# toverainc/willow-inference-server

Measured on AMD Instinct MI355X. Metric: realtime_multiple (audio_ms / infer_ms), Whisper large-v2 beam=5, 3.84 s clip, higher is better.
Workload: dtype f16; 1 GPU; whisper-large beam=5 clip=3sec (3840 ms) batch=1/GPU, PCM resident in HBM -> ids on host; parallelism=1 independent replicas (utterance sharding, no data-path collective)

## Files before the change

### include/wis_hip.h

```cpp
#ifndef WIS_HIP_H
#define WIS_HIP_H

#include <stddef.h>
#include <stdint.h>

#ifdef __cplusplus
extern "C" {
#endif

#define WIS_ABI_VERSION 1

#define WIS_OK             0
#define WIS_E_ARG         -1
#define WIS_E_FORMAT      -2
#define WIS_E_NOMEM       -3
#define WIS_E_CHECKSUM    -4
#define WIS_E_HIP         -5
#define WIS_E_STATE       -6
#define WIS_E_UNSUPPORTED -7

#define WIS_SAMPLE_RATE 16000
#define WIS_N_FFT       400
#define WIS_HOP         160
#define WIS_N_MELS      80
// ... 118 lines not shown
int wis_debug_align_matrix(wis_model_t* m, const float* input, int input_kind, int B, const int32_t* start_seq, int P,
                           const int32_t* text, const int32_t* text_len, const int32_t* num_frames, int median_filter_width, float* out);
int wis_align_last_timing(wis_model_t* m, float* ms);
int wis_op_dtw(int device, const float* x, int N, int M, int32_t* text_idx, int32_t* time_idx, int32_t* len);
int wis_op_align_matrix(int device, const float* q, const void* kx_f16, int T_tokens, int n_heads_sel, int T, int frames, int width, float* out);
int wis_debug_tree_logits(wis_model_t* m, const float* input, int input_kind, const int32_t* prompt, int P, int beam,
                          const int32_t* tok, const int32_t* org, int n_steps, float* logits);

int wis_debug_search(wis_model_t* m, const float* logits, int n_steps, int B, const wis_gen_opts_t* opts,
                     int32_t* out_ids, int32_t* out_len, float* out_score, int32_t* out_finish_step, int32_t* out_parent);
int wis_debug_search_n(wis_model_t* m, const float* logits, int n_steps, int B, const wis_gen_opts_t* opts, const uint64_t* seeds, const uint32_t* noise,
                       int32_t* out_ids, int32_t* out_len, float* out_score, int32_t* out_finish_step, int32_t* out_parent);

int wis_debug_handoff(wis_model_t* m, int raise_flag, int* retries, int* spin_disabled);
int wis_debug_graph_count(wis_model_t* m, int* count);
int wis_debug_sa_long(wis_model_t* m, int form);

typedef struct {
  float logmel_ms, encoder_ms, crosskv_ms, prefill_ms, decode_ms, total_ms;
  int32_t decode_steps;
  int32_t decode_steps_needed;
} wis_timing_t;
int wis_last_timing(const wis_model_t* m, wis_timing_t* t);

int wis_debug_phase_cycles(wis_model_t* m, int B, int beam, int pos, uint64_t* out);

int wis_debug_timeline(wis_model_t* m, int B, int beam, int pos, int use_graph, uint64_t* out, int n_out);
int wis_debug_sampling_cycles(wis_model_t* m, uint64_t* out);

int wis_bench_weight_stream(wis_model_t* m, int M, int passes, float* total_ms, int* launches_per_pass,
// ... 105 lines not shown
```

### willow-inference-server_amd/csrc/generate.hip

```cpp
#include <math.h>
#include <stdlib.h>
#include <string.h>
#include <time.h>
#include <algorithm>
#include <chrono>
#include <cmath>
#include <vector>

#include "common.hpp"
#include "kernels.hpp"
#include "model.hpp"

using namespace wis;

namespace {

struct SampleCtx {
  wis_model* m; hipStream_t st;
  int B, P, beam;
  SampleCfg sc; const float* bias_all;
  bool ts; int ts_max_init;
  float rep_pen = 1.f; int rep_ngram = 0;
  bool rep() const { return rep_pen != 1.f || rep_ngram != 0; }
  SampleP sp;
// ... 106 lines not shown
      for (int r = 0; r < B * beam; ++r) { ht[r] = r; ht[MAX_ROWS + r] = r / beam * beam; }
      WIS_HIP_CHECK(hipMemcpyAsync(m->d_sa_tab, ht, sizeof(m->h_pin->sa_tab), hipMemcpyHostToDevice, g.st));
    }
  } else
  if (!g.drafting || g.beam_draft) {
    std::vector<int> tok(B * P), pos(B * P), slot(B * P), ls(B * P);
    for (int b = 0; b < B; ++b) for (int i = 0; i < P; ++i) { tok[b * P + i] = g.prompt[b * P + i]; pos[b * P + i] = i; slot[b * P + i] = b * beam; ls[b * P + i] = b * beam; }
    WIS_RET(upload_rows(m, tok, pos, slot, ls, false));
  }
  if (m->overrun_left) { WIS_HIP_CHECK(hipMemsetAsync(m->ca_epoch, 0, 4, g.st)); m->overrun_left = false; }
  __atomic_store_n(&m->h_prog[HP_REC], 0ull, __ATOMIC_RELAXED);
  m->h_prog[HP_DONE_STEP] = 0; m->h_prog[HP_DONE_STAMP] = 0; m->h_prog[HP_STAMP0] = 0;
  return WIS_OK;
}

static int front_half(const GenCtx& g) {
  wis_model* m = g.m; hipStream_t st = g.st; const int B = g.B;
  static const bool one_stream = getenv("WIS_ONE_STREAM") != nullptr;
  static const bool two_streams = getenv("WIS_TWO_STREAMS") != nullptr;
  const bool alone = g_active_calls[m->device & 63].load(std::memory_order_relaxed) <= 1;
  hipStream_t se = (one_stream || !(alone || two_streams)) ? st : m->st_enc;
  if (se != st) WIS_HIP_CHECK(hipStreamWaitEvent(se, m->ev_ckv, 0));
  WIS_HIP_CHECK(hipEventRecord(m->ev[0], se));
  WIS_RET(stage_input(m, g.input, g.o->input_kind, B, se));
  WIS_HIP_CHECK(hipEventRecord(m->ev[1], se));
  WIS_RET(run_encoder(m, B, se));
  WIS_HIP_CHECK(hipEventRecord(m->ev[2], se));
  if (se != st) { WIS_HIP_CHECK(hipEventRecord(m->ev_enc, se)); WIS_HIP_CHECK(hipStreamWaitEvent(st, m->ev_enc, 0)); }
  WIS_RET(run_cross_kv(m, B));
  WIS_HIP_CHECK(hipEventRecord(m->ev[3], st));
  WIS_HIP_CHECK(hipEventRecord(m->ev_ckv, st));
  return WIS_OK;
}

struct LogitRows { int b, j, off; };
enum { TAIL_TAPS = 1, TAIL_NO_CACHE = 2 };
static int sampling_tail(const SampleCtx& g, LogitRows rows, int flags) {
  wis_model* m = g.m; hipStream_t st = g.st; const wis_config_t& c = m->cfg;
  const int lr_b = rows.b, lr_j = rows.j, lr_off = rows.off;
  unsigned long long* prof = (WIS_TAPS && (flags & TAIL_TAPS)) ? m->d_prof + (size_t)c.n_dec_layers * 8 * 16 : nullptr;
  if (g.rep()) WIS_RET(launch_rep_rules(st, m->logits, m->bs, g.B, g.sc, g.rep_pen, g.rep_ngram, lr_b, lr_j, lr_off));
  if (g.ts) WIS_RET(launch_ts_rules(st, m->logits, g.bias_all, m->bias_begin, m->bs, g.B, g.sc, c.no_timestamps, g.ts_max_init, lr_b, lr_j, lr_off, m->ts_desc));
  if (g.sampling()) {
    WIS_RET(launch_logit_stats(st, m->logits, g.bias_all, m->bias_begin, m->bs.step_u, m->st_max, m->st_sum, m->st_val, m->st_idx, g.B, g.sc, lr_b, lr_j, lr_off, nullptr,
// ... 22 lines not shown
  explicit TicketScope(wis_model* mm) : m(mm), spin_call(mm->spin_now) { m->spin_now = false; }
  ~TicketScope() { m->spin_now = spin_call; }
};

static int reseed_tick(wis_model* m, int steps) {
  unsigned* tk = m->h_pin->reseed_tick;
  tk[0] = (unsigned)steps; tk[1] = m->gen; tk[2] = 0; tk[3] = 0;
  WIS_HIP_CHECK(hipMemcpyAsync(m->bs.tick, tk, 16, hipMemcpyHostToDevice, m->st));
  return WIS_OK;
}

static void pack_traj(int* hd, const int32_t* tok, const int32_t* org, int n, int k) {
  for (int s_ = 0; s_ < n; ++s_) for (int j = 0; j < k; ++j) { hd[(s_ * MAX_R + j) * 2] = tok[s_ * k + j]; hd[(s_ * MAX_R + j) * 2 + 1] = org[s_ * k + j]; }
}

static int seed_prefill(const GenCtx& g) {
  wis_model* m = g.m; const wis_config_t& c = m->cfg; const int B = g.B, P = g.P;
  WIS_RET(dec_forward(m, B * P, P, B, true, g.beam, 0));
  if (g.sot_row >= 0) WIS_RET(launch_no_speech(g.st, m->logits, m->n_vocab_pad, B, P, g.sot_row, c.n_vocab, c.no_speech, m->d_nsp));
  return sampling_tail(g, {P, 0, P - 1}, TAIL_TAPS);
}

static int seed_prefill_long(const GenCtx& g) {
  wis_model* m = g.m; hipStream_t st = g.st; const wis_config_t& c = m->cfg; PinnedScratch* hp = m->h_pin;
  const int B = g.B, P = g.P, beam = g.beam, Pl = g.Pl, Np = P - Pl, G = MAX_ROWS / 16;
  for (int ub0 = 0; ub0 < B; ub0 += G) {
    const int nb = std::min(G, B - ub0), M = nb * 16;
    for (int r = 0; r < M; ++r) hp->base[r] = hp->anc[r] = (ub0 + r / 16) * beam;
    WIS_HIP_CHECK(hipMemcpyAsync(m->d_anc, hp->anc, (size_t)M * 4, hipMemcpyHostToDevice, st));
    WIS_HIP_CHECK(hipMemcpyAsync(m->d_base, hp->base, (size_t)M * 4, hipMemcpyHostToDevice, st));
    for (int t0 = 0; t0 < Np; t0 += 16) {
      const int n = std::min(16, Np - t0);
      std::vector<int> tok(M), pos(M), slot(M), ls(M);
      for (int r = 0; r < M; ++r) {
        const int u = ub0 + r / 16, i = std::min(r % 16, n - 1);
// ... 174 lines not shown
  ~StepGraph() { g.m->sa_nb = 8; }

  int nb_for(int passes_done) const {
    static const bool sa_short = !(getenv("WIS_SA_NB") && atoi(getenv("WIS_SA_NB")) == 0);
    const int len = g.P + passes_done;
    return (!sa_short || g.long_p) ? 8 : (len <= 16 ? 2 : (len <= 32 ? 4 : 8));
  }
  int one_step() const {
    g.m->sa_plen = g.plen; g.m->sa_w0 = g.P;
    const int rc = dec_forward(g.m, g.B * g.beam, g.beam, g.B, true, g.beam, 1);
    g.m->sa_plen = nullptr;
    WIS_RET(rc);
    return sampling_tail(g, {g.beam, 1, 0}, TAIL_TAPS | (g.sampling() ? TAIL_NO_CACHE : 0));
  }
  int graph_for(int nb, hipGraphExec_t* out) const {
    wis_model* m = g.m; const SampleCfg& sc = g.sc;
    GraphKey key; memset(&key, 0, sizeof(key));
    key.B = g.B; key.beam = g.beam; key.P = (g.long_p && sa_long_kernel(m)) ? -1 : g.P ; key.max_new = g.max_new; key.fixed_new = sc.fixed_new; key.suppress_blank = sc.suppress_blank;
    key.suppress_default = g.o->suppress_default; key.early_exit = sc.allow_early_exit; key.lp = sc.length_penalty; key.patience = g.patience; key.spin = m->spin_now ? 1 : 0;
    key.sa_nb = nb;
    key.timestamps = g.ts ? 1 : 0; key.max_init = g.ts ? g.ts_max_init : 0;
    key.rep_pen = g.rep_pen == 1.f ? 0.f : g.rep_pen; key.rep_ngram = g.rep_ngram;
    key.samp_topk = g.sp.topk; key.samp_T = g.sampling() ? g.sp.T : 0.f; key.n_hyp = g.n_res > 1 ? g.n_res : 0;
    auto it = m->graphs.find(key);
    if (it != m->graphs.end()) { *out = it->second; return WIS_OK; }
    hipGraph_t graph = nullptr; hipGraphExec_t ge = nullptr;
    WIS_HIP_CHECK(hipStreamBeginCapture(g.st, hipStreamCaptureModeThreadLocal));
    int rc = one_step();
    hipError_t e = hipStreamEndCapture(g.st, &graph);
    if (rc) { if (graph) hipGraphDestroy(graph); return rc; }
    if (e != hipSuccess) { set_error("graph capture failed: %s", hipGetErrorString(e)); return WIS_E_HIP; }
    e = hipGraphInstantiate(&ge, graph, nullptr, nullptr, 0);
    hipGraphDestroy(graph);
    if (e != hipSuccess) { set_error("graph instantiate failed: %s", hipGetErrorString(e)); return WIS_E_HIP; }
    m->graphs[key] = ge;
    *out = ge;
    return WIS_OK;
  }
// ... 1 lines not shown
    wis_model* m = g.m;
    m->sa_nb = nb_for(passes_done);
    if (!m->use_graph) return one_step();
    hipGraphExec_t ge = nullptr;
    WIS_RET(graph_for(m->sa_nb, &ge));
    WIS_HIP_CHECK(hipGraphLaunch(ge, g.st));
    return WIS_OK;
  }
};

struct LoopResult {
  int steps;
  int needed = 0;
  bool gave_up = false;
  bool from_host = false;
  float decode_ms_dev = -1.f;
};
static void unpack_progress(const wis_model* m, int* st_, int* dn_, int* gu_) {
  const unsigned long long r = __atomic_load_n(&m->h_prog[HP_REC], __ATOMIC_ACQUIRE);
  if ((r >> 48) != (unsigned long long)m->gen) { *st_ = 0; *dn_ = 0; *gu_ = 0; return; }
  *st_ = (int)((r >> 32) & 0xFFFFu); *gu_ = (int)((r >> 16) & 0xFFFFu); *dn_ = (int)(r & 0xFFFFu);
}
static int check_terminated(const GenCtx& g, LoopResult* lr, int dn_, int gu_) {
  lr->gave_up = gu_ != 0;
  if (!lr->gave_up && dn_ < g.B) { set_error("decode did not terminate within %d steps (done %d of %d)", lr->steps, dn_, g.B); return WIS_E_STATE; }
  return WIS_OK;
}

static inline void cpu_relax() {
#if !defined(__HIP_DEVICE_COMPILE__) && defined(__x86_64__)
  __builtin_ia32_pause();
#endif
}

static int run_burst(const GenCtx& g, const StepGraph& sg, int limit, LoopResult* lr) {
  wis_model* m = g.m;
  for (; lr->steps < limit; ++lr->steps) WIS_RET(sg.launch_pass(lr->steps));
  WIS_HIP_CHECK(hipEventRecord(m->ev[5], g.st));
  WIS_HIP_CHECK(hipStreamSynchronize(g.st));
  int st_, dn_, gu_; unpack_progress(m, &st_, &dn_, &gu_);
  WIS_RET(check_terminated(g, lr, dn_, gu_));
  lr->needed = lr->steps;
  return WIS_OK;
}

static int run_paced(const GenCtx& g, const StepGraph& sg, int limit, int base_done, LoopResult* lr) {
  wis_model* m = g.m; const int B = g.B;
  int& steps = lr->steps;
  const auto t_dec0 = std::chrono::steady_clock::now();
  const int depth = g.o->queue_depth > 0 ? g.o->queue_depth : 2;
  auto t_last = std::chrono::steady_clock::now();
  int seen = -1, st_ = 0, dn_ = 0, gu_ = 0;
  static const bool trace = getenv("WIS_EOT_TRACE") != nullptr;
  struct Tr { int step; unsigned long long dev; double host_us; int launched; };
  std::vector<Tr> tr;
  const auto t_loop = std::chrono::steady_clock::now();
  for (unsigned spins = 0;; ++spins) {
// ... 19 lines not shown
    }
    cpu_relax();
  }
  if (trace) {
    unsigned long long prev_dev = 0;
    for (size_t i = 0; i < tr.size(); ++i) {
      if (tr[i].step < 0) { fprintf(stderr, "[eot-trace]   launch of step %d took the host %.1f us\n", -tr[i].step, tr[i].host_us); continue; }
      fprintf(stderr, "[eot-trace] step %d seen by the host at %.1f us (device clock +%.1f us since the previous record), %d steps enqueued\n", tr[i].step, tr[i].host_us,
              prev_dev ? (double)(tr[i].dev - prev_dev) * 0.01 : 0.0, tr[i].launched);
      prev_dev = tr[i].dev;
    }
    fprintf(stderr, "[eot-trace] done seen at %.1f us: %d of %d utterances, %d steps enqueued\n", std::chrono::duration<double, std::micro>(std::chrono::steady_clock::now() - t_loop).count(), dn_, B, steps);
  }
  WIS_RET(check_terminated(g, lr, dn_, gu_));
  if (!lr->gave_up) {
    lr->from_host = true;
    lr->needed = (int)m->h_prog[HP_DONE_STEP];
    const unsigned long long s0 = m->h_prog[HP_STAMP0], s1 = m->h_prog[HP_DONE_STAMP];
    lr->decode_ms_dev = s1 > s0 ? (float)((double)(s1 - s0) * 1e-5) : 0.f;
    if (g.drafting) lr->decode_ms_dev = std::chrono::duration<float, std::milli>(std::chrono::steady_clock::now() - t_dec0).count();
  }
  return WIS_OK;
}

static void results_from_verification(const GenCtx& g, const Seed& sd, int32_t* out_ids, int32_t* out_len, float* out_score) {
  float sfin = sd.spec_cum;
  if (g.sc.length_penalty != 0.f) sfin /= powf((float)sd.spec_len, g.sc.length_penalty);
  out_len[0] = sd.spec_len;
  for (int t = 0; t < g.max_new; ++t) out_ids[t] = t < sd.spec_len ? sd.spec_gen[t] : 0;
  if (out_score) out_score[0] = sfin;
}
// ... 39 lines not shown
  m->timing.decode_steps_needed = lr.needed;
}

static int generate_impl(wis_model_t* m, const float* input, int B, const int32_t* prompt, int P,
                 const wis_gen_opts_t* o, int32_t* out_ids, int32_t* out_len, float* out_score, bool* retry,
                 const int32_t* draft = nullptr, int n_draft = 0, int* accepted = nullptr, const int32_t* draft_org = nullptr,
                 const uint64_t* seeds = nullptr, bool single = true) {
  *retry = false;
  if (accepted) *accepted = 0;
  m->nsp_B = 0;
  WIS_HIP_CHECK(hipSetDevice(m->device));
  SpinClaim claim(m, B);
  GenCtx g;
  WIS_RET(make_gen_ctx(m, input, B, prompt, P, o, draft, n_draft, draft_org, seeds, single, &g));
  hipStream_t st = g.st;
  WIS_RET(stage_search(g));
  WIS_RET(front_half(g));

  Seed sd;
  if (g.long_p) WIS_RET(seed_prefill_long(g));
  else if (!g.drafting) WIS_RET(seed_prefill(g));
  else {
    TicketScope ticket(m);
    WIS_RET(g.beam_draft ? seed_beam_draft(g, &sd) : seed_greedy_draft(g, &sd));
    if (accepted) *accepted = sd.accepted;
  }
  WIS_HIP_CHECK(hipEventRecord(m->ev[4], st));
  if (sd.beam_fin) WIS_HIP_CHECK(hipEventRecord(m->ev[5], st));

  const StepGraph sg{g};
  LoopResult lr; lr.steps = sd.steps;
  const int known = (g.sc.fixed_new > 0) ? std::min(g.max_new, g.sc.fixed_new + 1) : 0;
  if (sd.spec_done || sd.beam_fin) lr.needed = sd.steps;
  else if (known) WIS_RET(run_burst(g, sg, known, &lr));
  else WIS_RET(run_paced(g, sg, g.max_new, g.drafting ? sd.steps : 0, &lr));
  if (lr.gave_up) {
    WIS_HIP_CHECK(hipMemsetAsync(m->ca_epoch, 0, 4, st));
    WIS_HIP_CHECK(hipStreamSynchronize(st));
    m->spin_off = true; *retry = true; ++m->handoff_retries;
    fprintf(stderr, "[wis_hip] device %d: decoder cross-attention granule hand-off timed out; this handle uses the ticket hand-off from now on, the call is repeated\n", m->device);
    return WIS_OK;
  }
  if (sd.spec_done) { results_from_verification(g, sd, out_ids, out_len, out_score); lr.from_host = true; lr.decode_ms_dev = 0.f; }
  else if (lr.from_host) WIS_RET(results_from_record(g, out_ids, out_len, out_score));
  else WIS_RET(results_from_device(m, B * g.n_res, g.max_new, out_ids, out_len, out_score));
  record_timing(g, lr);
  if (lr.steps > lr.needed) { claim.defer(st); m->overrun_left = true; }
  if (g.sot_row >= 0) m->nsp_B = B;
  return WIS_OK;
}

static int generate_with_retry(const char* who, wis_model_t* m, const float* input, int B, const int32_t* prompt, int P, const wis_gen_opts_t* o,
                               int32_t* out_ids, int32_t* out_len, float* out_score,
                               const int32_t* draft = nullptr, int n_draft = 0, int* accepted = nullptr, const int32_t* draft_org = nullptr,
                               const uint64_t* seeds = nullptr, bool single = true) {
  bool retry = false;
  for (int attempt = 0; attempt < 2; ++attempt) {
    WIS_RET(generate_impl(m, input, B, prompt, P, o, out_ids, out_len, out_score, &retry, draft, n_draft, accepted, draft_org, seeds, single));
    if (!retry) return WIS_OK;
// ... 152 lines not shown
```

### willow-inference-server_amd/csrc/model.hip

```cpp
#include <math.h>
#include <stdlib.h>
#include <string.h>
#include <algorithm>
#include <atomic>
#include <mutex>
#include <memory>
#include <string>
#include <vector>

#include "common.hpp"
#include "kernels.hpp"
#include "model.hpp"

using namespace wis;

namespace wis {

__global__ void convert_kernel(const void* __restrict__ src, int src_f16, void* __restrict__ dst, int dst_f16,
                               int64_t rows, int64_t cols, int64_t dst_ld, int64_t n_scale, float scale) {
  const int64_t total = rows * cols;
  for (int64_t i = (int64_t)blockIdx.x * blockDim.x + threadIdx.x; i < total; i += (int64_t)gridDim.x * blockDim.x) {
    const int64_t r = i / cols, c = i - r * cols;
    float v = src_f16 ? (float)reinterpret_cast<const f16*>(src)[i] : reinterpret_cast<const float*>(src)[i];
    if (r < n_scale) v *= scale;
// ... 487 lines not shown
      const float* b = last ? m->enc_ln_b : m->enc[l + 1].ln1_b;
      WIS_RET(launch_gemm_splitk_resid(st, gemm_plain(m->hbuf, 4 * d, w.w_f2, M, d, 4 * d), splits, m->skbuf, w.b_f2, m->x, m->x, g, b, last ? m->mem : m->xn));
      xn_ready = true;
    } else {
      WIS_RET(launch_gemm_generic(st, gemm_plain(m->hbuf, 4 * d, w.w_f2, M, d, 4 * d), w.b_f2, m->x, m->x, 2 | 4));
    }
  }
  if (!split) WIS_RET(launch_layernorm(st, m->x, m->enc_ln_g, m->enc_ln_b, m->mem, M, d));
  return WIS_OK;
}
int run_cross_kv(wis_model* m, int B) {
  const wis_config_t& c = m->cfg;
  const int d = c.d_model, T = c.n_audio_ctx;
  return launch_gemm_crosskv(m->st, gemm_plain(m->mem, d, m->w_ckv_all, B * T, c.n_dec_layers * 2 * d, d), m->b_ckv_all, m->kx_all, m->vx_all, d, T, m->Tpad,
                             c.n_heads, (int64_t)m->kx_lstride, (int64_t)m->vx_lstride);
}

std::atomic<int> g_spin_bh[64];
struct DeferredClaim { hipEvent_t ev; int n; };
std::mutex g_spin_mu;
std::vector<DeferredClaim> g_spin_deferred[64];
static void spin_collect(int device) {
  std::lock_guard<std::mutex> lk(g_spin_mu);
  auto& v = g_spin_deferred[device & 63];
  for (size_t i = 0; i < v.size();) {
    if (hipEventQuery(v[i].ev) != hipErrorNotReady) { g_spin_bh[device & 63].fetch_sub(v[i].n, std::memory_order_relaxed); v[i] = v.back(); v.pop_back(); }
    else ++i;
  }
}
SpinClaim::SpinClaim(wis_model* mm, int B) : m(mm) {
// ... 305 lines not shown

int wis_model_create(const wis_config_t* cfg, const void* arena, size_t arena_bytes, int arena_on_device,
                     const wis_tensor_t* tensors, int n_tensors, int device, wis_model_t** out) {
  if (!cfg || !arena || !tensors || !out || n_tensors <= 0) { set_error("wis_model_create: bad argument"); return WIS_E_ARG; }
  if (cfg->d_model % 128 || cfg->d_model != cfg->n_heads * 64 || cfg->d_model > 2048 || !mel_bins_supported(cfg->n_mels) || cfg->n_enc_layers < 1 || cfg->n_dec_layers < 1 || cfg->n_audio_ctx != 1500 ||
      cfg->n_text_ctx > 512 || cfg->max_batch < 1 || cfg->max_beam < 1 || cfg->max_beam > MAX_R || cfg->n_vocab < 1024) {
    set_error("wis_model_create: unsupported config (d_model %% 128, head_dim 64, n_mels 80 or 128, n_audio_ctx 1500, max_beam <= %d)", MAX_R);
    return WIS_E_UNSUPPORTED;
  }
  DeviceCtx* ctx; WIS_RET(get_ctx(device, &ctx));
  wis_model* m = new wis_model();
  m->cfg = *cfg; m->device = device; m->ctx = ctx;
  m->w8 = cfg->decoder_weight_bits == 8;
  m->cq_fold = !m->w8 && getenv("WIS_NO_CQFOLD") == nullptr;
  m->use_graph = getenv("WIS_NO_GRAPH") == nullptr;
  memset(&m->timing, 0, sizeof(m->timing));
  int rc = WIS_OK;
  void* d_arena = nullptr;
  do {
    if (hipStreamCreateWithFlags(&m->st, hipStreamNonBlocking) != hipSuccess) { set_error("stream create failed"); rc = WIS_E_HIP; break; }
    const char* base = reinterpret_cast<const char*>(arena);
    if (!arena_on_device) {
      if (hipMalloc(&d_arena, arena_bytes) != hipSuccess) { set_error("hipMalloc(arena %zu) failed", arena_bytes); rc = WIS_E_NOMEM; break; }
      if (hipMemcpy(d_arena, arena, arena_bytes, hipMemcpyHostToDevice) != hipSuccess) { set_error("arena upload failed"); rc = WIS_E_HIP; break; }
      base = reinterpret_cast<const char*>(d_arena);
    }
    Loader L{tensors, n_tensors, base, arena_bytes};
    if ((rc = load_weights(m, L))) break;
    {
      std::vector<float> ba(m->n_vocab_pad, 0.f), bb(m->n_vocab_pad, 0.f);
// ... 11 lines not shown
    m->slab_cur = nullptr; m->slab_left = 0;
    if ((rc = alloc_buffers(m))) break;
    if (hipStreamSynchronize(m->st) != hipSuccess) { set_error("model init failed"); rc = WIS_E_HIP; break; }
  } while (0);
  if (d_arena) hipFree(d_arena);
  if (rc) { wis_model_destroy(m); return rc; }
  *out = m;
  return WIS_OK;
}

void wis_model_destroy(wis_model_t* m) {
  if (!m) return;
  hipSetDevice(m->device);
  if (m->st) hipStreamSynchronize(m->st);
  spin_collect(m->device);
  for (auto& kv : m->graphs) hipGraphExecDestroy(kv.second);
  for (void* p : m->allocs) hipFree(p);
  if (m->h_pin) hipHostFree(m->h_pin);
  if (m->h_prog) hipHostFree(m->h_prog);
  for (int i = 0; i < 8; ++i) if (m->ev[i]) hipEventDestroy(m->ev[i]);
  for (hipEvent_t e : m->al.ev) if (e) hipEventDestroy(e);
  if (m->st_enc) { hipStreamSynchronize(m->st_enc); hipStreamDestroy(m->st_enc); }
  if (m->ev_enc) hipEventDestroy(m->ev_enc);
  if (m->ev_ckv) hipEventDestroy(m->ev_ckv);
  if (m->st) hipStreamDestroy(m->st);
  delete m;
}
size_t wis_model_device_bytes(const wis_model_t* m) { return m ? m->bytes : 0; }

int wis_model_clone(wis_model_t* parent, wis_model_t** out) {
  if (!parent || !out || !parent->wslabs) { set_error("wis_model_clone: bad argument"); return WIS_E_ARG; }
  WIS_HIP_CHECK(hipSetDevice(parent->device));
  wis_model* m = new wis_model();
  m->cfg = parent->cfg; m->device = parent->device; m->ctx = parent->ctx;
  m->wslabs = parent->wslabs;
  m->w_conv1 = parent->w_conv1; m->w_conv2 = parent->w_conv2; m->b_conv1 = parent->b_conv1; m->b_conv2 = parent->b_conv2;
  m->enc_pos = parent->enc_pos; m->enc_ln_g = parent->enc_ln_g; m->enc_ln_b = parent->enc_ln_b;
  m->enc = parent->enc; m->dec = parent->dec;
  m->emb = parent->emb; m->dec_pos = parent->dec_pos; m->proj = parent->proj; m->dec_ln_g = parent->dec_ln_g; m->dec_ln_b = parent->dec_ln_b;
  m->bias_all = parent->bias_all; m->bias_begin = parent->bias_begin; m->d_lang_ids = parent->d_lang_ids; m->n_vocab_pad = parent->n_vocab_pad;
  m->w_ckv_all = parent->w_ckv_all; m->b_ckv_all = parent->b_ckv_all;
  m->w8 = parent->w8; m->cq_fold = parent->cq_fold;
  m->use_graph = parent->use_graph;
  m->al.heads = parent->al.heads;
  memset(&m->timing, 0, sizeof(m->timing));
  int rc = WIS_OK;
  do {
    if (hipStreamCreateWithFlags(&m->st, hipStreamNonBlocking) != hipSuccess) { set_error("stream create failed"); rc = WIS_E_HIP; break; }
    if ((rc = alloc_buffers(m))) break;
    if (hipStreamSynchronize(m->st) != hipSuccess) { set_error("clone init failed"); rc = WIS_E_HIP; break; }
  } while (0);
  if (rc) { wis_model_destroy(m); return rc; }
  *out = m;
  return WIS_OK;
}

int wis_last_no_speech_prob(wis_model_t* m, int B, float* out) {
  if (!m || !out || B < 1) { set_error("wis_last_no_speech_prob: bad argument"); return WIS_E_ARG; }
// ... 22 lines not shown
  for (int s = 0; s < n; ++s) for (int j = 0; j < k; ++j) { tok[s * k + j] = raw[((size_t)s * MAX_R + j) * 2]; org[s * k + j] = raw[((size_t)s * MAX_R + j) * 2 + 1]; }
  *n_steps = n;
  return WIS_OK;
}

int wis_debug_sa_long(wis_model_t* m, int form) {
  if (!m || form < -1 || form > 1) { set_error("wis_debug_sa_long: bad argument"); return WIS_E_ARG; }
  WIS_ENTER(m, "wis_debug_sa_long")
  m->sa_long_form = form;
  return WIS_OK;
}
int wis_debug_graph_count(wis_model_t* m, int* count) {
  if (!m || !count) { set_error("wis_debug_graph_count: bad argument"); return WIS_E_ARG; }
  WIS_ENTER(m, "wis_debug_graph_count")
  *count = (int)m->graphs.size();
  return WIS_OK;
}
int wis_debug_handoff(wis_model_t* m, int raise_flag, int* retries, int* spin_disabled) {
  if (!m) { set_error("wis_debug_handoff: bad argument"); return WIS_E_ARG; }
  WIS_ENTER(m, "wis_debug_handoff")
  WIS_HIP_CHECK(hipSetDevice(m->device));
  if (raise_flag) {
    const unsigned one = 1u;
    WIS_HIP_CHECK(hipMemcpyAsync(m->ca_epoch, &one, 4, hipMemcpyHostToDevice, m->st));
    WIS_HIP_CHECK(hipStreamSynchronize(m->st));
  }
  if (retries) *retries = m->handoff_retries;
  if (spin_disabled) *spin_disabled = m->spin_off ? 1 : 0;
  return WIS_OK;
}
// ... 31 lines not shown
```

### willow-inference-server_amd/csrc/model.hpp

```cpp
#pragma once
#include <string.h>
#include <array>
#include <atomic>
#include <map>
#include <memory>
#include <vector>

#include "common.hpp"
#include "kernels.hpp"

namespace wis {

struct EncLayerW {
  float *ln1_g, *ln1_b, *ln2_g, *ln2_b;
  f16 *w_qkv, *w_out, *w_f1, *w_f2;
  float *b_qkv, *b_out, *b_f1, *b_f2;
};
struct DecProj {
  const f16* Wp;
  const float* scale;
  const float* bias;
  const float* csum;
  int N, K;
  int rows;
  const f16* Wp8 = nullptr;
};
struct DecLayerW {
  float *ln1_g, *ln1_b, *ln2_g, *ln2_b, *ln3_g, *ln3_b;
  DecProj qkv, out, cq, cout, f1, f2;
  DecProj cqo;
  f16* w_ckv; float* b_ckv;
  std::array<const DecProj*, 6> streamed() const { return {&qkv, &out, &cq, &cout, &f1, &f2}; }
};

struct GraphKey {
  int B, beam, P, max_new, fixed_new, suppress_blank, suppress_default, early_exit, spin, sa_nb; float lp, patience;
  int timestamps, max_init;
  float rep_pen; int rep_ngram;
  int samp_topk; float samp_T; int n_hyp;
  bool operator<(const GraphKey& o) const { return memcmp(this, &o, sizeof(GraphKey)) < 0; }
};

struct WeightSlabs {
  int device; std::vector<void*> slabs; size_t bytes = 0;
  ~WeightSlabs() { hipSetDevice(device); for (void* p : slabs) hipFree(p); }
};

struct AlignState {
  std::vector<int> heads;
  bool ready = false;
  bool capture = false;
  int nsel = 0, sel_cap = 0; size_t sel_bytes = 0;
  std::vector<int> layer_s0;
  int* d_sel_head = nullptr; long long* d_koff = nullptr;
  f16* qsel = nullptr;
  float *W = nullptr, *acc = nullptr;
// ... 80 lines not shown
  int nsp_B = 0;
  float* d_in; int64_t* d_nsamp; float* d_probs;
  int* vstep = nullptr; int* pick_tok = nullptr; float* pick_lp = nullptr;
  int* d_draft = nullptr; int* d_anc = nullptr; int* d_vstate = nullptr; int* d_base = nullptr;
  float* lm_logspec = nullptr; unsigned* lm_gmax = nullptr;
  wis::PinnedScratch* h_pin = nullptr;
  unsigned long long* h_prog = nullptr;
  unsigned gen = 0;
  int last_B = 0, last_beam = 0;
  bool overrun_left = false;
  hipEvent_t ev[8];
  hipStream_t st_enc = nullptr;
  hipEvent_t ev_enc = nullptr, ev_ckv = nullptr;
  wis_timing_t timing;
  std::map<wis::GraphKey, hipGraphExec_t> graphs;
  bool use_graph;
  bool w8 = false;
  bool cq_fold = false;
  wis::f16* dxh = nullptr;
  unsigned long long* d_prof;
  bool prof_on; bool prof_all;
  size_t enc_part_cap = 0;
  std::atomic_flag busy = ATOMIC_FLAG_INIT;
  wis::AlignState al;
};

namespace wis {

extern std::atomic<int> g_active_calls[64];
struct BusyGuard {
  wis_model* m; bool ok;
  explicit BusyGuard(wis_model* mm) : m(mm), ok(!mm->busy.test_and_set(std::memory_order_acquire)) { if (ok) g_active_calls[m->device & 63].fetch_add(1, std::memory_order_relaxed); }
  ~BusyGuard() { if (ok) { g_active_calls[m->device & 63].fetch_sub(1, std::memory_order_relaxed); m->busy.clear(std::memory_order_release); } }
};
#define WIS_ENTER(m, what)                                                                                      \
  ::wis::BusyGuard _busy(m);                                                                                    \
  if (!_busy.ok) { ::wis::set_error("%s: another call is running on this handle (one call at a time per replica)", what); return WIS_E_STATE; }

int check_batch(wis_model* m, int B, int beam);
int stage_input(wis_model* m, const float* input, int kind, int B, hipStream_t on = nullptr);
int run_encoder(wis_model* m, int B, hipStream_t on = nullptr);
int run_cross_kv(wis_model* m, int B);
int conv1_k(int n_mels);
GemmP conv1_gemm(const f16* img, const f16* w, int B, int T, int n_mels, int N);
GemmP conv2_gemm(const f16* c1, const f16* w, int B, int T, int cin, int N);
void pack_conv1_w(hipStream_t st, const void* src, int src_f16, f16* dst, int N, int n_mels);
void pack_conv2_w(hipStream_t st, const void* src, int src_f16, f16* dst, int N, int cin);
int launch_mel_to_image(hipStream_t st, const float* mel, f16* img, int B, int n_mels);
int enc_splitk(int d, int M);
void launch_convert(hipStream_t st, const void* src, int src_f16, void* dst, int dst_f16, int64_t rows, int64_t cols, int64_t dst_ld, int64_t n_scale, float scale);
void launch_f16_to_f32(hipStream_t st, const f16* s, float* d, int64_t n);

int prep_projection(hipStream_t st, f16* W, int N, int Npad, int K, int n_scale, float scale, const float* gamma, const float* beta, float* bias, float* csum,
                    void* out, float* scale_out, int rows);
int build_cq_fold(hipStream_t st, const f16* wq_gamma, const void* wo, int wo_f16, const float* bo, int d, float qs, f16* fcat, f16* fwot, f16* fwqo, f16* p_cqo, float* b_cqo);

// ... 35 lines not shown
```

### willow-inference-server_amd/csrc/taps.hip

```cpp
#include <string.h>
#include <algorithm>
#include <vector>

#include "common.hpp"
#include "kernels.hpp"
#include "model.hpp"
#include "tap.hpp"

using namespace wis;

extern "C" {

int wis_debug_encode(wis_model_t* m, const float* input, int input_kind, int B, float* enc_out) {
  if (!m || !input || !enc_out) { set_error("wis_debug_encode: bad argument"); return WIS_E_ARG; }
  WIS_ENTER(m, "wis_debug_encode")
  WIS_HIP_CHECK(hipSetDevice(m->device));
  WIS_RET(check_batch(m, B, 1));
  WIS_RET(stage_input(m, input, input_kind, B));
  WIS_RET(run_encoder(m, B));
  const int64_t n = (int64_t)B * m->cfg.n_audio_ctx * m->cfg.d_model;
  launch_f16_to_f32(m->st, m->mem, m->x, n);
  WIS_HIP_CHECK(hipMemcpyAsync(enc_out, m->x, (size_t)n * 4, hipMemcpyDeviceToHost, m->st));
  WIS_HIP_CHECK(hipStreamSynchronize(m->st));
  return WIS_OK;
}

static int debug_logits_rows(const char* who, wis_model_t* m, const float* input, int input_kind, int B, const int32_t* dec_in, int T, int R, float* logits) {
  WIS_ENTER(m, who)
  WIS_HIP_CHECK(hipSetDevice(m->device));
  WIS_RET(check_batch(m, B, 1));
  if (B * R > MAX_ROWS) { set_error("%s: B*R = %d exceeds %d decoder rows per pass", who, B * R, MAX_ROWS); return WIS_E_STATE; }
  WIS_RET(stage_input(m, input, input_kind, B));
  WIS_RET(run_encoder(m, B));
  WIS_RET(run_cross_kv(m, B));
// ... 567 lines not shown
```

### willow-inference-server_amd/wis_hip/_lib.py

```python
import ctypes as C
import os

import numpy as np

_HERE = os.path.dirname(os.path.abspath(__file__))
LIB_PATH = os.environ.get("WIS_LIB_PATH") or os.path.join(os.path.dirname(_HERE), "lib", "libwis_hip.so")

WIS_OK = 0
WIS_IN_MEL_HOST, WIS_IN_MEL_DEV, WIS_IN_PCM_HOST, WIS_IN_PCM_DEV = 0, 1, 2, 3
WIS_DT_F32, WIS_DT_F16 = 0, 1
N_SAMPLES, N_FRAMES, N_MELS = 480000, 3000, 80


class WisError(RuntimeError):
    def __init__(self, code, msg):
        super().__init__(f"libwis_hip error {code}: {msg}")
        self.code = code


class Config(C.Structure):
    _fields_ = [(n, C.c_int32) for n in ("d_model", "n_heads", "n_enc_layers", "n_dec_layers", "n_vocab", "n_audio_ctx",
                                          "n_text_ctx", "n_mels", "max_batch", "max_beam", "eot", "sot", "no_timestamps",
                                          "no_speech")] + [
        ("suppress_ids", C.POINTER(C.c_int32)), ("n_suppress", C.c_int32),
# ... 70 lines not shown
    ("wis_debug_logits", _i, [_vp, _vp, _i, _i, C.POINTER(C.c_int32), _i, _fp]),
    ("wis_debug_logits_rows", _i, [_vp, _vp, _i, _i, C.POINTER(C.c_int32), _i, _i, _fp]),
    ("wis_model_set_alignment_heads", _i, [_vp, C.POINTER(C.c_int32), _i]),
    ("wis_align", _i, [_vp, _vp, _i, _i, C.POINTER(C.c_int32), _i, C.POINTER(C.c_int32), C.POINTER(C.c_int32), C.POINTER(C.c_int32), _i,
                       C.POINTER(C.c_int32), C.POINTER(C.c_int32), C.POINTER(C.c_int32), _fp]),
    ("wis_debug_align_matrix", _i, [_vp, _vp, _i, _i, C.POINTER(C.c_int32), _i, C.POINTER(C.c_int32), C.POINTER(C.c_int32), C.POINTER(C.c_int32), _i, _fp]),
    ("wis_align_last_timing", _i, [_vp, _fp]),
    ("wis_op_dtw", _i, [_i, _vp, _i, _i, _vp, _vp, _vp]),
    ("wis_op_align_matrix", _i, [_i, _vp, _vp, _i, _i, _i, _i, _i, _vp]),
    ("wis_debug_tree_logits", _i, [_vp, _vp, _i, C.POINTER(C.c_int32), _i, _i, C.POINTER(C.c_int32), C.POINTER(C.c_int32), _i, _fp]),
    ("wis_debug_search", _i, [_vp, _vp, _i, _i, C.POINTER(GenOpts), C.POINTER(C.c_int32), C.POINTER(C.c_int32), _fp, C.POINTER(C.c_int32), C.POINTER(C.c_int32)]),
    ("wis_debug_search_n", _i, [_vp, _vp, _i, _i, C.POINTER(GenOpts), C.POINTER(C.c_uint64), C.POINTER(C.c_uint32), C.POINTER(C.c_int32), C.POINTER(C.c_int32), _fp,
                                C.POINTER(C.c_int32), C.POINTER(C.c_int32)]),
    ("wis_debug_handoff", _i, [_vp, _i, C.POINTER(_i), C.POINTER(_i)]),
    ("wis_debug_graph_count", _i, [_vp, C.POINTER(_i)]),
    ("wis_debug_sa_long", _i, [_vp, _i]),
    ("wis_last_timing", _i, [_vp, C.POINTER(Timing)]),
    ("wis_debug_phase_cycles", _i, [_vp, _i, _i, _i, C.POINTER(C.c_uint64)]),
    ("wis_debug_timeline", _i, [_vp, _i, _i, _i, _i, C.POINTER(C.c_uint64), _i]),
    ("wis_debug_sampling_cycles", _i, [_vp, C.POINTER(C.c_uint64)]),
    ("wis_bench_weight_stream", _i, [_vp, _i, _i, _fp, C.POINTER(_i), C.POINTER(C.c_double)]),
    ("wis_dev_alloc", _i, [_i, _sz, C.POINTER(_vp)]),
    ("wis_dev_free", _i, [_i, _vp]),
    ("wis_dev_h2d", _i, [_i, _vp, _vp, _sz]),
    ("wis_dev_d2h", _i, [_i, _vp, _vp, _sz]),
    ("wis_dev_sync", _i, [_i]),
    ("wis_dev_copy_peer", _i, [_i, _vp, _i, _vp, _sz]),
    ("wis_op_gemm", _i, [_i, _vp, _i, _vp, _vp, _vp, _vp, _i, _i, _i, _i]),
    ("wis_op_layernorm", _i, [_i, _vp, _vp, _vp, _vp, _i, _i]),
    ("wis_op_enc_attention", _i, [_i, _vp, _vp, _vp, _i, _i, _i, _i]),
# ... 111 lines not shown
```

Baseline: 150.5 x realtime.

## Capture encoder and prefill into HIP graphs and launch encoder before search staging

Wraps the encoder chain and the prefill pass (decoder forward plus sampling tail) in cached HIP graphs, keyed by batch and by an extended graph key, so these many small kernel launches become a single graph launch per call. The encoder launch is also moved ahead of search staging, so the host setup work overlaps with encoder execution, and the cross-KV wait is split into its own step. Results are read from the record whenever decode finished in-record, not only on the host path. This adds graph-cache memory and a capture cost on first use, falls back to per-kernel launches if capture fails, and can be disabled with WIS_FRONT_GRAPH=0.

```diff
diff --git a/include/wis_hip.h b/include/wis_hip.h
--- a/include/wis_hip.h
+++ b/include/wis_hip.h
@@ -156,6 +156,7 @@
 
 int wis_debug_handoff(wis_model_t* m, int raise_flag, int* retries, int* spin_disabled);
 int wis_debug_graph_count(wis_model_t* m, int* count);
+int wis_debug_front_graph_count(wis_model_t* m, int* count);
 int wis_debug_sa_long(wis_model_t* m, int form);
 
 typedef struct {
diff --git a/willow-inference-server_amd/csrc/generate.hip b/willow-inference-server_amd/csrc/generate.hip
--- a/willow-inference-server_amd/csrc/generate.hip
+++ b/willow-inference-server_amd/csrc/generate.hip
@@ -144,7 +144,7 @@
   return WIS_OK;
 }
 
-static int front_half(const GenCtx& g) {
+static int front_encoder(const GenCtx& g, hipStream_t* enc_stream) {
   wis_model* m = g.m; hipStream_t st = g.st; const int B = g.B;
   static const bool one_stream = getenv("WIS_ONE_STREAM") != nullptr;
   static const bool two_streams = getenv("WIS_TWO_STREAMS") != nullptr;
@@ -154,10 +154,16 @@
   WIS_HIP_CHECK(hipEventRecord(m->ev[0], se));
   WIS_RET(stage_input(m, g.input, g.o->input_kind, B, se));
   WIS_HIP_CHECK(hipEventRecord(m->ev[1], se));
-  WIS_RET(run_encoder(m, B, se));
+  WIS_RET(launch_encoder(m, B, se));
   WIS_HIP_CHECK(hipEventRecord(m->ev[2], se));
-  if (se != st) { WIS_HIP_CHECK(hipEventRecord(m->ev_enc, se)); WIS_HIP_CHECK(hipStreamWaitEvent(st, m->ev_enc, 0)); }
-  WIS_RET(run_cross_kv(m, B));
+  if (se != st) WIS_HIP_CHECK(hipEventRecord(m->ev_enc, se));
+  *enc_stream = se;
+  return WIS_OK;
+}
+static int front_cross_kv(const GenCtx& g, hipStream_t se) {
+  wis_model* m = g.m; hipStream_t st = g.st;
+  if (se != st) WIS_HIP_CHECK(hipStreamWaitEvent(st, m->ev_enc, 0));
+  WIS_RET(run_cross_kv(m, g.B));
   WIS_HIP_CHECK(hipEventRecord(m->ev[3], st));
   WIS_HIP_CHECK(hipEventRecord(m->ev_ckv, st));
   return WIS_OK;
@@ -210,11 +216,39 @@
   for (int s_ = 0; s_ < n; ++s_) for (int j = 0; j < k; ++j) { hd[(s_ * MAX_R + j) * 2] = tok[s_ * k + j]; hd[(s_ * MAX_R + j) * 2 + 1] = org[s_ * k + j]; }
 }
 
-static int seed_prefill(const GenCtx& g) {
+static int prefill_pass(const GenCtx& g) {
   wis_model* m = g.m; const wis_config_t& c = m->cfg; const int B = g.B, P = g.P;
   WIS_RET(dec_forward(m, B * P, P, B, true, g.beam, 0));
   if (g.sot_row >= 0) WIS_RET(launch_no_speech(g.st, m->logits, m->n_vocab_pad, B, P, g.sot_row, c.n_vocab, c.no_speech, m->d_nsp));
   return sampling_tail(g, {P, 0, P - 1}, TAIL_TAPS);
+}
+
+static GraphKey pass_key(const GenCtx& g, int kind, int sa_nb) {
+  const wis_model* m = g.m; const SampleCfg& sc = g.sc;
+  GraphKey key; memset(&key, 0, sizeof(key));
+  key.B = g.B; key.beam = g.beam; key.P = (g.long_p && sa_long_kernel(m)) ? -1 : g.P ; key.max_new = g.max_new; key.fixed_new = sc.fixed_new; key.suppress_blank = sc.suppress_blank;
+  key.suppress_default = g.o->suppress_default; key.early_exit = sc.allow_early_exit; key.lp = sc.length_penalty; key.patience = g.patience; key.spin = m->spin_now ? 1 : 0;
+  key.sa_nb = sa_nb;
+  key.timestamps = g.ts ? 1 : 0; key.max_init = g.ts ? g.ts_max_init : 0;
+  key.rep_pen = g.rep_pen == 1.f ? 0.f : g.rep_pen; key.rep_ngram = g.rep_ngram;
+  key.samp_topk = g.sp.topk; key.samp_T = g.sampling() ? g.sp.T : 0.f; key.n_hyp = g.n_res > 1 ? g.n_res : 0;
+  key.kind = kind; key.sot_row = kind == GRAPH_PREFILL ? g.sot_row : 0;
+  return key;
+}
+
+static int seed_prefill(const GenCtx& g) {
+  wis_model* m = g.m;
+  if (!m->front_graph) return prefill_pass(g);
+  const GraphKey key = pass_key(g, GRAPH_PREFILL, 8);
+  auto it = m->graphs.find(key);
+  if (it == m->graphs.end()) {
+    hipGraphExec_t ge = nullptr;
+    WIS_RET(capture_chain(m, g.st, "prefill pass", [&] { return prefill_pass(g); }, &ge));
+    it = m->graphs.emplace(key, ge).first;
+  }
+  if (!it->second) return prefill_pass(g);
+  WIS_HIP_CHECK(hipGraphLaunch(it->second, g.st));
+  return WIS_OK;
 }
 
 static int seed_prefill_long(const GenCtx& g) {
@@ -419,14 +453,8 @@
     return sampling_tail(g, {g.beam, 1, 0}, TAIL_TAPS | (g.sampling() ? TAIL_NO_CACHE : 0));
   }
   int graph_for(int nb, hipGraphExec_t* out) const {
-    wis_model* m = g.m; const SampleCfg& sc = g.sc;
-    GraphKey key; memset(&key, 0, sizeof(key));
-    key.B = g.B; key.beam = g.beam; key.P = (g.long_p && sa_long_kernel(m)) ? -1 : g.P ; key.max_new = g.max_new; key.fixed_new = sc.fixed_new; key.suppress_blank = sc.suppress_blank;
-    key.suppress_default = g.o->suppress_default; key.early_exit = sc.allow_early_exit; key.lp = sc.length_penalty; key.patience = g.patience; key.spin = m->spin_now ? 1 : 0;
-    key.sa_nb = nb;
-    key.timestamps = g.ts ? 1 : 0; key.max_init = g.ts ? g.ts_max_init : 0;
-    key.rep_pen = g.rep_pen == 1.f ? 0.f : g.rep_pen; key.rep_ngram = g.rep_ngram;
-    key.samp_topk = g.sp.topk; key.samp_T = g.sampling() ? g.sp.T : 0.f; key.n_hyp = g.n_res > 1 ? g.n_res : 0;
+    wis_model* m = g.m;
+    const GraphKey key = pass_key(g, GRAPH_STEP, nb);
     auto it = m->graphs.find(key);
     if (it != m->graphs.end()) { *out = it->second; return WIS_OK; }
     hipGraph_t graph = nullptr; hipGraphExec_t ge = nullptr;
@@ -458,6 +486,7 @@
   int needed = 0;
   bool gave_up = false;
   bool from_host = false;
+  bool in_record = false;
   float decode_ms_dev = -1.f;
 };
 static void unpack_progress(const wis_model* m, int* st_, int* dn_, int* gu_) {
@@ -485,6 +514,7 @@
   int st_, dn_, gu_; unpack_progress(m, &st_, &dn_, &gu_);
   WIS_RET(check_terminated(g, lr, dn_, gu_));
   lr->needed = lr->steps;
+  lr->in_record = !lr->gave_up;
   return WIS_OK;
 }
 
@@ -534,7 +564,7 @@
   }
   WIS_RET(check_terminated(g, lr, dn_, gu_));
   if (!lr->gave_up) {
-    lr->from_host = true;
+    lr->from_host = lr->in_record = true;
     lr->needed = (int)m->h_prog[HP_DONE_STEP];
     const unsigned long long s0 = m->h_prog[HP_STAMP0], s1 = m->h_prog[HP_DONE_STAMP];
     lr->decode_ms_dev = s1 > s0 ? (float)((double)(s1 - s0) * 1e-5) : 0.f;
@@ -604,8 +634,10 @@
   GenCtx g;
   WIS_RET(make_gen_ctx(m, input, B, prompt, P, o, draft, n_draft, draft_org, seeds, single, &g));
   hipStream_t st = g.st;
+  hipStream_t se = nullptr;
+  WIS_RET(front_encoder(g, &se));
   WIS_RET(stage_search(g));
-  WIS_RET(front_half(g));
+  WIS_RET(front_cross_kv(g, se));
 
   Seed sd;
   if (g.long_p) WIS_RET(seed_prefill_long(g));
@@ -632,7 +664,7 @@
     return WIS_OK;
   }
   if (sd.spec_done) { results_from_verification(g, sd, out_ids, out_len, out_score); lr.from_host = true; lr.decode_ms_dev = 0.f; }
-  else if (lr.from_host) WIS_RET(results_from_record(g, out_ids, out_len, out_score));
+  else if (lr.in_record) WIS_RET(results_from_record(g, out_ids, out_len, out_score));
   else WIS_RET(results_from_device(m, B * g.n_res, g.max_new, out_ids, out_len, out_score));
   record_timing(g, lr);
   if (lr.steps > lr.needed) { claim.defer(st); m->overrun_left = true; }
diff --git a/willow-inference-server_amd/csrc/model.hip b/willow-inference-server_amd/csrc/model.hip
--- a/willow-inference-server_amd/csrc/model.hip
+++ b/willow-inference-server_amd/csrc/model.hip
@@ -525,6 +525,43 @@
   const int d = c.d_model, T = c.n_audio_ctx;
   return launch_gemm_crosskv(m->st, gemm_plain(m->mem, d, m->w_ckv_all, B * T, c.n_dec_layers * 2 * d, d), m->b_ckv_all, m->kx_all, m->vx_all, d, T, m->Tpad,
                              c.n_heads, (int64_t)m->kx_lstride, (int64_t)m->vx_lstride);
+}
+
+int capture_chain(wis_model* m, hipStream_t st, const char* what, const std::function<int()>& enqueue, hipGraphExec_t* out) {
+  *out = nullptr;
+  hipGraph_t graph = nullptr; hipGraphExec_t ge = nullptr;
+  hipError_t e = hipStreamBeginCapture(st, hipStreamCaptureModeThreadLocal);
+  const char* stage = "begin capture";
+  if (e == hipSuccess) {
+    const int rc = enqueue();
+    e = hipStreamEndCapture(st, &graph);
+    if (rc) { if (graph) hipGraphDestroy(graph); (void)hipGetLastError(); return rc; }
+    stage = "end capture";
+    if (e == hipSuccess) { e = hipGraphInstantiate(&ge, graph, nullptr, nullptr, 0); stage = "instantiate"; }
+    if (graph) hipGraphDestroy(graph);
+  }
+  if (e != hipSuccess) {
+    (void)hipGetLastError();
+    if (!m->graph_fallback_logged) {
+      m->graph_fallback_logged = true;
+      fprintf(stderr, "[wis_hip] device %d: graph of the %s not available (%s: %s); launched kernel by kernel instead\n", m->device, what, stage, hipGetErrorString(e));
+    }
+    return WIS_OK;
+  }
+  *out = ge;
+  return WIS_OK;
+}
+int launch_encoder(wis_model* m, int B, hipStream_t on) {
+  if (!m->front_graph) return run_encoder(m, B, on);
+  auto it = m->enc_graphs.find(B);
+  if (it == m->enc_graphs.end()) {
+    hipGraphExec_t ge = nullptr;
+    WIS_RET(capture_chain(m, on, "encoder", [&] { return run_encoder(m, B, on); }, &ge));
+    it = m->enc_graphs.emplace(B, ge).first;
+  }
+  if (!it->second) return run_encoder(m, B, on);
+  WIS_HIP_CHECK(hipGraphLaunch(it->second, on));
+  return WIS_OK;
 }
 
 std::atomic<int> g_spin_bh[64];
@@ -860,6 +897,7 @@
   m->w8 = cfg->decoder_weight_bits == 8;
   m->cq_fold = !m->w8 && getenv("WIS_NO_CQFOLD") == nullptr;
   m->use_graph = getenv("WIS_NO_GRAPH") == nullptr;
+  { const char* e = getenv("WIS_FRONT_GRAPH"); m->front_graph = m->use_graph && !(e && atoi(e) == 0); }
   memset(&m->timing, 0, sizeof(m->timing));
   int rc = WIS_OK;
   void* d_arena = nullptr;
@@ -901,7 +939,8 @@
   hipSetDevice(m->device);
   if (m->st) hipStreamSynchronize(m->st);
   spin_collect(m->device);
-  for (auto& kv : m->graphs) hipGraphExecDestroy(kv.second);
+  for (auto& kv : m->graphs) if (kv.second) hipGraphExecDestroy(kv.second);
+  for (auto& kv : m->enc_graphs) if (kv.second) hipGraphExecDestroy(kv.second);
   for (void* p : m->allocs) hipFree(p);
   if (m->h_pin) hipHostFree(m->h_pin);
   if (m->h_prog) hipHostFree(m->h_prog);
@@ -928,7 +967,7 @@
   m->bias_all = parent->bias_all; m->bias_begin = parent->bias_begin; m->d_lang_ids = parent->d_lang_ids; m->n_vocab_pad = parent->n_vocab_pad;
   m->w_ckv_all = parent->w_ckv_all; m->b_ckv_all = parent->b_ckv_all;
   m->w8 = parent->w8; m->cq_fold = parent->cq_fold;
-  m->use_graph = parent->use_graph;
+  m->use_graph = parent->use_graph; m->front_graph = parent->front_graph;
   m->al.heads = parent->al.heads;
   memset(&m->timing, 0, sizeof(m->timing));
   int rc = WIS_OK;
@@ -981,6 +1020,15 @@
   if (!m || !count) { set_error("wis_debug_graph_count: bad argument"); return WIS_E_ARG; }
   WIS_ENTER(m, "wis_debug_graph_count")
   *count = (int)m->graphs.size();
+  return WIS_OK;
+}
+int wis_debug_front_graph_count(wis_model_t* m, int* count) {
+  if (!m || !count) { set_error("wis_debug_front_graph_count: bad argument"); return WIS_E_ARG; }
+  WIS_ENTER(m, "wis_debug_front_graph_count")
+  int n = 0;
+  for (auto& kv : m->graphs) n += kv.first.kind == GRAPH_PREFILL && kv.second;
+  for (auto& kv : m->enc_graphs) n += kv.second != nullptr;
+  *count = n;
   return WIS_OK;
 }
 int wis_debug_handoff(wis_model_t* m, int raise_flag, int* retries, int* spin_disabled) {
diff --git a/willow-inference-server_amd/csrc/model.hpp b/willow-inference-server_amd/csrc/model.hpp
--- a/willow-inference-server_amd/csrc/model.hpp
+++ b/willow-inference-server_amd/csrc/model.hpp
@@ -2,6 +2,7 @@
 #include <string.h>
 #include <array>
 #include <atomic>
+#include <functional>
 #include <map>
 #include <memory>
 #include <vector>
@@ -38,8 +39,11 @@
   int timestamps, max_init;
   float rep_pen; int rep_ngram;
   int samp_topk; float samp_T; int n_hyp;
+  int kind, sot_row;
   bool operator<(const GraphKey& o) const { return memcmp(this, &o, sizeof(GraphKey)) < 0; }
 };
+
+enum { GRAPH_STEP = 0, GRAPH_PREFILL = 1 };
 
 struct WeightSlabs {
   int device; std::vector<void*> slabs; size_t bytes = 0;
@@ -150,7 +154,10 @@
   hipEvent_t ev_enc = nullptr, ev_ckv = nullptr;
   wis_timing_t timing;
   std::map<wis::GraphKey, hipGraphExec_t> graphs;
+  std::map<int, hipGraphExec_t> enc_graphs;
   bool use_graph;
+  bool front_graph = false;
+  bool graph_fallback_logged = false;
   bool w8 = false;
   bool cq_fold = false;
   wis::f16* dxh = nullptr;
@@ -176,6 +183,8 @@
 int check_batch(wis_model* m, int B, int beam);
 int stage_input(wis_model* m, const float* input, int kind, int B, hipStream_t on = nullptr);
 int run_encoder(wis_model* m, int B, hipStream_t on = nullptr);
+int launch_encoder(wis_model* m, int B, hipStream_t on);
+int capture_chain(wis_model* m, hipStream_t st, const char* what, const std::function<int()>& enqueue, hipGraphExec_t* out);
 int run_cross_kv(wis_model* m, int B);
 int conv1_k(int n_mels);
 GemmP conv1_gemm(const f16* img, const f16* w, int B, int T, int n_mels, int N);
diff --git a/willow-inference-server_amd/csrc/taps.hip b/willow-inference-server_amd/csrc/taps.hip
--- a/willow-inference-server_amd/csrc/taps.hip
+++ b/willow-inference-server_amd/csrc/taps.hip
@@ -17,7 +17,7 @@
   WIS_HIP_CHECK(hipSetDevice(m->device));
   WIS_RET(check_batch(m, B, 1));
   WIS_RET(stage_input(m, input, input_kind, B));
-  WIS_RET(run_encoder(m, B));
+  WIS_RET(launch_encoder(m, B, m->st));
   const int64_t n = (int64_t)B * m->cfg.n_audio_ctx * m->cfg.d_model;
   launch_f16_to_f32(m->st, m->mem, m->x, n);
   WIS_HIP_CHECK(hipMemcpyAsync(enc_out, m->x, (size_t)n * 4, hipMemcpyDeviceToHost, m->st));
diff --git a/willow-inference-server_amd/wis_hip/_lib.py b/willow-inference-server_amd/wis_hip/_lib.py
--- a/willow-inference-server_amd/wis_hip/_lib.py
+++ b/willow-inference-server_amd/wis_hip/_lib.py
@@ -108,6 +108,7 @@
                                 C.POINTER(C.c_int32), C.POINTER(C.c_int32)]),
     ("wis_debug_handoff", _i, [_vp, _i, C.POINTER(_i), C.POINTER(_i)]),
     ("wis_debug_graph_count", _i, [_vp, C.POINTER(_i)]),
+    ("wis_debug_front_graph_count", _i, [_vp, C.POINTER(_i)]),
     ("wis_debug_sa_long", _i, [_vp, _i]),
     ("wis_last_timing", _i, [_vp, C.POINTER(Timing)]),
     ("wis_debug_phase_cycles", _i, [_vp, _i, _i, _i, C.POINTER(C.c_uint64)]),
```

Result: no change. 150.8 x realtime (median of 6 runs) (+0.2%).
